# gnosisguild/stylus-zkvm-verifiers

Hardware: AMD Instinct MI355X
Metric: Groth16 proofs verified/sec (BN254) (higher is better)
Workload: dtype u32

## Files before the change

### stylus_zkvm_verifiers_amd/csrc/zkv_field.h

```cpp
#pragma once
#include <stdint.h>
#include "bn254_constants.h"

#if defined(__HIPCC__)
#define ZKV_HD __host__ __device__ __forceinline__
#define ZKV_HD_NI __host__ __device__ __noinline__ inline
#else
#define ZKV_HD inline
#define ZKV_HD_NI inline
#endif

#if defined(ZKV_COUNT_FP_MUL)
static thread_local unsigned long long zkv_fp_mul_counter = 0;
static thread_local unsigned long long zkv_mad_counter = 0;
static thread_local unsigned long long zkv_mad_issued_counter = 0;
static thread_local unsigned long long zkv_sqr_mad_excess_counter = 0;
#define ZKV_COUNT_MADS(n) (zkv_mad_counter += (n), zkv_mad_issued_counter += (n))
#define ZKV_COUNT_MADS_ISSUED(n) (zkv_mad_issued_counter += (n))
#else
#define ZKV_COUNT_MADS(n) ((void)0)
#define ZKV_COUNT_MADS_ISSUED(n) ((void)0)
#endif

#if defined(__HIP_DEVICE_COMPILE__)
#define ZKV_TABLE static __device__ const
#else
#define ZKV_TABLE static const
#endif

#if defined(ZKV_ASM_MARKS) && defined(__HIP_DEVICE_COMPILE__)
#define ZKV_MARK(name) asm volatile("; ZKVMARK " name)
#else
#define ZKV_MARK(name) ((void)0)
#endif

#ifndef ZKV_FAIR_SLICE_SHIFT
#define ZKV_FAIR_SLICE_SHIFT 17
#endif
ZKV_HD uint32_t zkv_wave_slot_parity() {
#if defined(__HIP_DEVICE_COMPILE__) && !defined(ZKV_NO_FAIR_SHARE)
    return __builtin_amdgcn_s_getreg((3 << 11) | 4) & 1u;
#else
    return 0;
#endif
}
ZKV_HD void zkv_fair_share(uint32_t slot_parity) {
#if defined(__HIP_DEVICE_COMPILE__) && !defined(ZKV_NO_FAIR_SHARE)
    const uint32_t t = (uint32_t)(__builtin_amdgcn_s_memrealtime() >> ZKV_FAIR_SLICE_SHIFT);
    if ((t ^ slot_parity) & 1u) __builtin_amdgcn_s_setprio(1);
    else __builtin_amdgcn_s_setprio(0);
#else
    (void)slot_parity;
#endif
}

#include "zkv_modinv.h"

namespace zkv {

struct Fp { uint32_t v[8]; };
struct Fp2C { Fp c0, c1; };
#if defined(ZKV_PAIRED)
struct Fp2 { Fp h; };
#else
struct Fp2 { Fp c0, c1; };
#endif
struct Fp6 { Fp2 c0, c1, c2; };

#if defined(__has_builtin)
#if __has_builtin(__builtin_addc) && __has_builtin(__builtin_subc)
#define ZKV_HAVE_CARRY_BUILTINS 1
#endif
#endif
ZKV_HD uint32_t addc(uint32_t a, uint32_t b, uint32_t& carry) {
#if defined(ZKV_HAVE_CARRY_BUILTINS)
    unsigned co; uint32_t r = __builtin_addc(a, b, carry, &co); carry = co; return r;
#else
    uint64_t t = (uint64_t)a + b + carry;
    carry = (uint32_t)(t >> 32);
    return (uint32_t)t;
#endif
}
ZKV_HD uint32_t subb(uint32_t a, uint32_t b, uint32_t& borrow) {
#if defined(ZKV_HAVE_CARRY_BUILTINS)
    unsigned bo; uint32_t r = __builtin_subc(a, b, borrow, &bo); borrow = bo; return r;
#else
    uint64_t t = (uint64_t)a - b - borrow;
    borrow = (uint32_t)(t >> 32) & 1u;
    return (uint32_t)t;
#endif
}

ZKV_HD Fp fp_zero() { Fp r; for (int i = 0; i < 8; i++) r.v[i] = 0; return r; }
ZKV_HD Fp fp_one() { Fp r = ZKV_FP_ONE; return r; }
ZKV_HD bool fp_is_zero(const Fp& a) {
    const uint32_t P[8] = ZKV_FP_P_LIMBS;
    uint32_t o = 0, q = 0;
    for (int i = 0; i < 8; i++) { o |= a.v[i]; q |= a.v[i] ^ P[i]; }
    return o == 0 || q == 0;
// ... 448 lines not shown
        if ((xo[i] >> 29) || (xp[i] >> 29) || (U[i] >> 29) || (V[i] >> 30)) zkv_col_shadow_bad++;
}
#define ZKV_DOT3_OPERANDS(a, b, c, d) zkv_dot3_operands(a, b, c, d)
#else
#define ZKV_DOT3_OPERANDS(a, b, c, d) ((void)0)
#endif
#if defined(ZKV_SHADOW_COLS) && !defined(__HIP_DEVICE_COMPILE__)
inline void zkv_limbs_below(const uint32_t (&a)[9], int bits) {
    for (int i = 0; i < 9; i++)
        if (a[i] >> bits) zkv_col_shadow_bad++;
}
#define ZKV_LIMBS_BELOW(a, bits) zkv_limbs_below(a, bits)
#else
#define ZKV_LIMBS_BELOW(a, bits) ((void)0)
#endif
ZKV_HD void f2_sum_open(uint64_t (&col)[18]) {
#pragma unroll
    for (int k = 0; k < 18; k++) col[k] = 0;
}
ZKV_HD void f2_sum_cross(uint64_t (&col)[18], const uint32_t (&ao)[9], const uint32_t (&ap)[9], const uint32_t (&bU)[9], const uint32_t (&bV)[9]) {
#if defined(ZKV_COUNT_FP_MUL)
    zkv_fp_mul_counter += 2;
#endif
    ZKV_DOT3_OPERANDS(ao, ap, bU, bV);
    fp_mac81(col, ao, bU); fp_mac81(col, ap, bV);
}
ZKV_HD void f2_sum_cross_dbl(uint64_t (&col)[18], const uint32_t (&ao2)[9], const uint32_t (&ap2)[9], const uint32_t (&bU)[9], const uint32_t (&bV)[9]) {
#if defined(ZKV_COUNT_FP_MUL)
    zkv_fp_mul_counter += 2;
#endif
    ZKV_LIMBS_BELOW(ao2, 30); ZKV_LIMBS_BELOW(ap2, 30); ZKV_LIMBS_BELOW(bU, 29); ZKV_LIMBS_BELOW(bV, 30);
    fp_mac81(col, ao2, bU); fp_mac81(col, ap2, bV);
}
ZKV_HD void f2_sum_sqr(uint64_t (&col)[18], const uint32_t (&M)[9], const uint32_t (&N)[9]) {
#if defined(ZKV_COUNT_FP_MUL)
    zkv_fp_mul_counter += 1;
#endif
    ZKV_LIMBS_BELOW(M, 30); ZKV_LIMBS_BELOW(N, 29);
    fp_mac81(col, M, N);
}
ZKV_HD Fp f2_sum_close(uint64_t (&col)[18]) {
    Fp r = fp_reduce_cols(col);
#if defined(__HIP_DEVICE_COMPILE__)
#pragma unroll
    for (int k = 0; k < 8; k++) asm volatile("" : "+v"(r.v[k]));
    __builtin_amdgcn_sched_barrier(0);
#endif
    return r;
}
ZKV_HD void fp_cols_carry32_dbl(uint64_t (&col)[18]) {
    uint32_t sixteen = 16u, two = 2u;
#if defined(__HIP_DEVICE_COMPILE__)
    asm volatile("" : "+s"(sixteen));
    asm volatile("" : "+s"(two));
#endif
#pragma unroll
    for (int k = 17; k >= 1; k--) {
        const uint32_t hi = (uint32_t)(col[k - 1] >> 32);
        const uint64_t keep = k == 17 ? col[17] + col[17] : (uint64_t)(uint32_t)col[k] * two;
        ZKV_COUNT_MADS_ISSUED(2);
        col[k] = col_add(keep, (uint64_t)hi * sixteen);
#if defined(__HIP_DEVICE_COMPILE__)
        asm volatile("" : "+v"(col[k]));
#endif
    }
    col[0] = (uint64_t)(uint32_t)col[0] * two;
}
ZKV_HD void f2_limbs_x_dbl(const Fp& v, uint32_t (&own2)[9], uint32_t (&par2)[9]) {
    uint32_t x[9];
    fp_unpack29(v, x);
#pragma unroll
    for (int i = 0; i < 9; i++) { own2[i] = x[i] << 1; par2[i] = zkv_partner_u32(own2[i]); }
}
ZKV_HD void f2_limbs_sqr(const uint32_t (&own)[9], const uint32_t (&par)[9], uint32_t (&M)[9], uint32_t (&N)[9]) {
    const uint32_t FAT[9] = ZKV_FP_FAT8P_LIMBS;
    const bool odd = zkv_parity() != 0;
#pragma unroll
    for (int i = 0; i < 9; i++) {
        M[i] = par[i] + (odd ? par[i] : own[i]);
        N[i] = own[i] + (odd ? 0u : FAT[i] - par[i]);
    }
#pragma unroll
    for (int k = 0; k < 8; k++) { N[k + 1] += N[k] >> 29; N[k] &= 0x1fffffffu; }
}
ZKV_HD void f2_dot3_first(uint64_t (&col)[18], const uint32_t (&ao)[9], const uint32_t (&ap)[9], const uint32_t (&bU)[9], const uint32_t (&bV)[9],
                          const uint32_t (&co)[9], const uint32_t (&cp)[9], const uint32_t (&dU)[9], const uint32_t (&dV)[9]) {
    f2_sum_open(col);
    f2_sum_cross(col, ao, ap, bU, bV); f2_sum_cross(col, co, cp, dU, dV);
    fp_cols_carry32(col);
}
ZKV_HD Fp f2_dot3_last(uint64_t (&col)[18], const uint32_t (&eo)[9], const uint32_t (&ep)[9], const uint32_t (&fU)[9], const uint32_t (&fV)[9]) {
    f2_sum_cross(col, eo, ep, fU, fV);
    return f2_sum_close(col);
}
ZKV_HD Fp f2_mul_limbs(const uint32_t (&ao)[9], const uint32_t (&ap)[9], const uint32_t (&bU)[9], const uint32_t (&bV)[9]) {
#if defined(ZKV_COUNT_FP_MUL)
    zkv_fp_mul_counter += 2;
#endif
    uint64_t col[18];
#pragma unroll
    for (int k = 0; k < 18; k++) col[k] = 0;
    fp_mac81(col, ao, bU); fp_mac81(col, ap, bV);
    return fp_reduce_cols(col);
}
struct L9 { uint32_t l[9]; };
ZKV_HD L9 l9_from_fp(const Fp& a) { L9 r; fp_unpack29(a, r.l); return r; }
ZKV_HD Fp l9_to_fp(const L9& a) { return fp_pack29(a.l); }
ZKV_HD L9 l9_partner(const L9& a) {
    L9 r;
#pragma unroll
    for (int i = 0; i < 9; i++) r.l[i] = zkv_partner_u32(a.l[i]);
    return r;
}
ZKV_HD L9 l9_mul_core(const L9& a, const L9& b) {
#if defined(ZKV_COUNT_FP_MUL)
    zkv_fp_mul_counter += 2;
#endif
    const uint32_t FAT[9] = ZKV_FP_FAT8P_LIMBS;
    uint32_t xo[9], U[9], V[9];
    uint64_t col[18];
#pragma unroll
    for (int k = 0; k < 18; k++) col[k] = 0;
#pragma unroll
    for (int i = 0; i < 9; i++) U[i] = zkv_pair_even_u32(b.l[i]);
    fp_mac81(col, a.l, U);
#pragma unroll
    for (int i = 0; i < 9; i++) { xo[i] = zkv_partner_u32(a.l[i]); V[i] = zkv_pair_odd_u32(b.l[i]); }
    if (zkv_parity() == 0) {
#pragma unroll
        for (int i = 0; i < 9; i++) V[i] = FAT[i] - V[i];
    }
    fp_mac81(col, xo, V);
    L9 r; fp_reduce_cols_limbs(col, r.l);
    return r;
}
#if defined(__HIP_DEVICE_COMPILE__) && defined(ZKV_FP_MUL_NOINLINE)
#define ZKV_L9P(p) uint32_t p##0, uint32_t p##1, uint32_t p##2, uint32_t p##3, uint32_t p##4, uint32_t p##5, uint32_t p##6, uint32_t p##7, uint32_t p##8
#define ZKV_L9A(f) f.l[0], f.l[1], f.l[2], f.l[3], f.l[4], f.l[5], f.l[6], f.l[7], f.l[8]
#define ZKV_L9MK(f, p) L9 f; f.l[0] = p##0; f.l[1] = p##1; f.l[2] = p##2; f.l[3] = p##3; f.l[4] = p##4; f.l[5] = p##5; f.l[6] = p##6; f.l[7] = p##7; f.l[8] = p##8
__device__ __noinline__ inline L9 l9_mul_ni(ZKV_L9P(pa), ZKV_L9P(pb)) {
    ZKV_L9MK(a, pa); ZKV_L9MK(b, pb);
    return l9_mul_core(a, b);
}
ZKV_HD L9 l9_mul(const L9& a, const L9& b) { return l9_mul_ni(ZKV_L9A(a), ZKV_L9A(b)); }
#else
ZKV_HD L9 l9_mul(const L9& a, const L9& b) { return l9_mul_core(a, b); }
#endif
struct LTerm { const uint32_t* x; int32_t k; };
#define ZKV_L9_G 256
template <int N> ZKV_HD L9 l9_lincomb(const LTerm (&t)[N], const int c) {
    const uint32_t P29[9] = ZKV_FP_P29_LIMBS;
    const int32_t D = (int32_t)P29[8] + 1;
    const uint32_t M = (uint32_t)(((1ull << 53) + (uint64_t)D - 1) / (uint64_t)D);
    int32_t top = 0;
#pragma unroll
    for (int j = 0; j < N; j++) top += t[j].k * (int32_t)t[j].x[8];
    const uint32_t tt = (uint32_t)(top + c * D - c - ZKV_L9_G);
    const int32_t nq = c - (int32_t)(uint32_t)(((uint64_t)tt * M) >> 53);
    L9 y; int64_t carry = 0;
#pragma unroll
    for (int i = 0; i < 9; i++) {
        int64_t s = carry;
#pragma unroll
        for (int j = 0; j < N; j++) s += (int64_t)t[j].k * (int64_t)(int32_t)t[j].x[i];
        s += (int64_t)nq * (int64_t)(int32_t)P29[i];
        if (i < 8) { y.l[i] = (uint32_t)s & 0x1fffffffu; carry = s >> 29; }
// ... 104 lines not shown
```

### stylus_zkvm_verifiers_amd/csrc/zkv_tower_mem.h

```cpp
#pragma once
#include "zkv_curve.h"

namespace zkv {

struct MRef {
    uint32_t* p; uint32_t stride; uint32_t f2w;
    ZKV_HD uint32_t ld(int k) const { return p[(size_t)k * stride]; }
    ZKV_HD void st(int k, uint32_t v) const { p[(size_t)k * stride] = v; }
    ZKV_HD int fw() const { return (int)f2w; }
};
ZKV_HD MRef m_ref(uint32_t* p, uint32_t stride, uint32_t f2w = 16) { MRef r; r.p = p; r.stride = stride; r.f2w = f2w; return r; }
ZKV_HD MRef m_off(MRef m, int words) { MRef r = m; r.p = m.p + (size_t)words * m.stride; return r; }

struct SoaRW {
    uint32_t* p; size_t stride; uint32_t off;
    ZKV_HD uint32_t ld(int k) const { return *(const uint32_t*)((const char*)(p + (size_t)k * stride) + off); }
    ZKV_HD void st(int k, uint32_t v) const { *(uint32_t*)((char*)(p + (size_t)k * stride) + off) = v; }
    ZKV_HD int fw() const { return 16; }
};
template <class R> ZKV_HD R m_fresh(R r) { return r; }
ZKV_HD SoaRW m_fresh(SoaRW r) {
#if defined(__HIP_DEVICE_COMPILE__)
    asm volatile("" : "+v"(r.off));
#endif
// ... 102 lines not shown
template <class RF> ZKV_HD void f12m_sqr_fused_body(RF f) {
    enum { A0 = 0, A1 = 3, A2 = 1, A3 = 4, A4 = 2, A5 = 5 };
    uint32_t x3o[9], x3p[9], y0U[9], y0V[9], z5U[9], z5V[9];
    uint32_t hU[9], hV[9];
    uint32_t ko[9], kp[9], jo[9], jp[9];
    uint32_t xo[9], xp[9], tU[9], tV[9];
    uint64_t col[18];
    Fp2 o1, o2, o3, o4, o5, o;
    f2_limbs_x(m_ld_f2(f, A3).h, x3o, x3p);
    f2_limbs_y(m_ld_f2(f, A1).h, hU, hV);
    f2_limbs_y(m_ld_f2(f, A2).h, tU, tV);
    f2_sum_open(col);
    f2_sum_cross(col, x3o, x3p, tU, tV);
    f2_limbs_x(m_ld_f2(f, A4).h, ko, kp);
    f2_sum_cross(col, ko, kp, hU, hV);
    fp_cols_carry32_dbl(col);
    f2_limbs_y(m_ld_f2(f, A0).h, y0U, y0V);
    f2_limbs_x_dbl(m_ld_f2(f, A5).h, xo, xp);
    f2_sum_cross_dbl(col, xo, xp, y0U, y0V);
    o5.h = f2_sum_close(col);
    f2_sum_open(col);
    f2_sum_cross(col, x3o, x3p, y0U, y0V);
    f2_limbs_x(m_ld_f2_again(f, A2).h, xo, xp);
    f2_sum_cross(col, xo, xp, hU, hV);
    fp_cols_carry32_dbl(col);
    { const Fp2 x5 = f2_mul_xi(m_ld_f2_again(f, A5)); f2_limbs_y(x5.h, z5U, z5V); }
    limbs_dbl_pinned(ko, kp, xo, xp);
    f2_sum_cross_dbl(col, xo, xp, z5U, z5V);
    o3.h = f2_sum_close(col);
    f2_sum_open(col);
    f2_sum_cross(col, ko, kp, y0U, y0V);
    f2_sum_cross(col, x3o, x3p, hU, hV);
    fp_cols_carry32_dbl(col);
    f2_limbs_x(m_ld_f2_again(f, A2).h, xo, xp);
    f2_limbs_sqr(xo, xp, tU, tV);
    f2_sum_sqr(col, tU, tV);
    f2_limbs_x(m_ld_f2_again(f, A5).h, xo, xp);
    f2_sum_cross(col, xo, xp, z5U, z5V);
    o4.h = f2_sum_close(col);
    m_st_f2(f, A5, o5);
    { const Fp2 x4 = f2_mul_xi(m_ld_f2_again(f, A4)); f2_limbs_y(x4.h, hU, hV); }
    f2_sum_open(col);
    f2_sum_cross(col, x3o, x3p, hU, hV);
    f2_limbs_x(m_ld_f2_again(f, A2).h, ko, kp);
    f2_sum_cross(col, ko, kp, z5U, z5V);
    fp_cols_carry32_dbl(col);
    f2_limbs_x(m_ld_f2_again(f, A1).h, jo, jp);
    limbs_dbl_pinned(jo, jp, xo, xp);
    f2_sum_cross_dbl(col, xo, xp, y0U, y0V);
    o1.h = f2_sum_close(col);
    f2_sum_open(col);
    f2_sum_cross(col, ko, kp, y0U, y0V);
    f2_sum_cross(col, x3o, x3p, z5U, z5V);
    fp_cols_carry32_dbl(col);
    f2_limbs_sqr(jo, jp, tU, tV);
    limbs_pin(tU); limbs_pin(tV);
    f2_sum_sqr(col, tU, tV);
    f2_limbs_x(m_ld_f2_again(f, A4).h, xo, xp);
    f2_sum_cross(col, xo, xp, hU, hV);
    o2.h = f2_sum_close(col);
    m_st_f2(f, A4, o4);
    f2_sum_open(col);
    f2_sum_cross(col, jo, jp, z5U, z5V);
    f2_sum_cross(col, ko, kp, hU, hV);
    fp_cols_carry32_dbl(col);
    f2_limbs_x(m_ld_f2_again(f, A0).h, xo, xp);
    f2_limbs_sqr(xo, xp, tU, tV);
    f2_sum_sqr(col, tU, tV);
    { const Fp2 x3 = f2_mul_xi(m_ld_f2_again(f, A3)); f2_limbs_y(x3.h, tU, tV); }
    f2_sum_cross(col, x3o, x3p, tU, tV);
    o.h = f2_sum_close(col);
    m_st_f2(f, A0, o); m_st_f2(f, A1, o1); m_st_f2(f, A2, o2); m_st_f2(f, A3, o3);
#if defined(ZKV_COUNT_FP_MUL)
    zkv_fp_mul_counter -= 15; zkv_mad_counter -= 729; zkv_mad_issued_counter -= 933; zkv_sqr_mad_excess_counter += 933;
#endif
}
template <class RF> ZKV_HD void f12m_sqr_body(RF f) {
#if defined(ZKV_SQR_KARATSUBA) && !defined(__HIP_DEVICE_COMPILE__)
    f12m_sqr_karatsuba_body(f);
#else
    f12m_sqr_fused_body(f);
#endif
}
#else
template <class RF> ZKV_HD void f12m_sqr_body(RF f) { f12m_sqr_karatsuba_body(f); }
#endif
template <class RF> ZKV_HD_NI void f12m_sqr(RF f) { f12m_sqr_body(f); }
ZKV_HD void fp4_sqr(const Fp2& a, const Fp2& b, Fp2& t0, Fp2& t1) {
    Fp2 tmp = f2_mul(a, b);
    t0 = f2_sub(f2_sub(f2_mul(f2_add(a, b), f2_add(f2_mul_xi(b), a)), tmp), f2_mul_xi(tmp));
    t1 = f2_dbl(tmp);
}
template <class RF> ZKV_HD void f12m_cyclo_sqr_body(RF f) {
    Fp2 z0 = m_ld_f2(f, 0), z1 = m_ld_f2(f, 4), t0, t1;
    fp4_sqr(z0, z1, t0, t1);
    z0 = f2_sub(t0, z0); z0 = f2_add(f2_dbl(z0), t0);
    z1 = f2_add(t1, z1); z1 = f2_add(f2_dbl(z1), t1);
    m_st_f2(f, 0, z0); m_st_f2(f, 4, z1);
    Fp2 z2 = m_ld_f2(f, 3), z3 = m_ld_f2(f, 2), t2, t3;
    fp4_sqr(z2, z3, t2, t3);
    Fp2 z4 = m_ld_f2(f, 1), z5 = m_ld_f2(f, 5), t4, t5;
    fp4_sqr(z4, z5, t4, t5);
    Fp2 x = f2_mul_xi(t5);
    z2 = f2_add(x, z2); z2 = f2_add(f2_dbl(z2), x);
    z3 = f2_sub(t4, z3); z3 = f2_add(f2_dbl(z3), t4);
    z4 = f2_sub(t2, z4); z4 = f2_add(f2_dbl(z4), t2);
    z5 = f2_add(t3, z5); z5 = f2_add(f2_dbl(z5), t3);
    m_st_f2(f, 3, z2); m_st_f2(f, 2, z3); m_st_f2(f, 1, z4); m_st_f2(f, 5, z5);
}
template <class RF> ZKV_HD_NI void f12m_cyclo_sqr(RF f) { f12m_cyclo_sqr_body(f); }
#if defined(ZKV_PAIRED)
struct L9Ref {
    zkv_lds_u32* p;
    ZKV_HD int fw() const { return 8; }
};
ZKV_HD L9Ref l9_ref(uint32_t* lds_base_plus_lane) { L9Ref r; r.p = (zkv_lds_u32*)lds_base_plus_lane; return r; }
ZKV_HD L9 l9_ld(L9Ref m, int idx) {
    L9 r;
#pragma unroll
    for (int k = 0; k < 9; k++) r.l[k] = m.p[(9 * idx + k) * 64];
    return r;
}
ZKV_HD void l9_st(L9Ref m, int idx, const L9& a) {
#pragma unroll
    for (int k = 0; k < 9; k++) m.p[(9 * idx + k) * 64] = a.l[k];
}
ZKV_HD Fp m_ld_fp(L9Ref m, int word0) { return l9_to_fp(l9_ld(m, word0 >> 3)); }
ZKV_HD void m_st_fp(L9Ref m, int word0, const Fp& a) { l9_st(m, word0 >> 3, l9_from_fp(a)); }

ZKV_HD void l9_fp4_sqr_update(const L9& a, const L9& b, const L9& za, const L9& zb, const bool xi_t1, L9& o0, L9& o1) {
    const bool odd = zkv_parity() != 0;
    const int32_t k1 = odd ? 1 : -1, k3 = odd ? -3 : 3;
    const L9 tmp = l9_mul(a, b);
    L9 s1, s2;
#pragma unroll
    for (int i = 0; i < 9; i++) s1.l[i] = a.l[i] + b.l[i];
    {
        const L9 pb = l9_partner(b);
        const LTerm t[3] = {{a.l, 1}, {b.l, 9}, {pb.l, k1}};
        s2 = l9_lincomb(t, 4);
    }
    const L9 S = l9_mul(s1, s2);
    const L9 tp = l9_partner(tmp);
    {
        const LTerm t[4] = {{S.l, 3}, {tmp.l, -30}, {tp.l, k3}, {za.l, -2}};
        o0 = l9_lincomb(t, 72);
    }
    if (!xi_t1) {
        const LTerm t[2] = {{tmp.l, 6}, {zb.l, 2}};
        o1 = l9_lincomb(t, 1);
    } else {
        const LTerm t[3] = {{tmp.l, 54}, {tp.l, -2 * k3}, {zb.l, 2}};
        o1 = l9_lincomb(t, 14);
    }
}
ZKV_HD void f12l9_cyclo_sqr(L9Ref f) {
    {
        const L9 a = l9_ld(f, 0), b = l9_ld(f, 4);
        L9 o0, o1;
        l9_fp4_sqr_update(a, b, a, b, false, o0, o1);
        l9_st(f, 0, o0); l9_st(f, 4, o1);
    }
    L9 n1, n5;
    {
        const L9 a = l9_ld(f, 3), b = l9_ld(f, 2), za = l9_ld(f, 1), zb = l9_ld(f, 5);
        l9_fp4_sqr_update(a, b, za, zb, false, n1, n5);
// ... 338 lines not shown
```

### stylus_zkvm_verifiers_amd/csrc/zkv_verify.h

```cpp
#pragma once
#include "zkv_tower_mem.h"
#include "zkv_sha256.h"
#include "zkv_gt.h"

namespace zkv {

enum : uint8_t {
    ST_OK = 0, ST_VERIFICATION_FAILED = 1, ST_INVALID_INITIALIZATION = 2, ST_ALREADY_INITIALIZED = 3,
    ST_INVALID_PROOF_DATA = 4, ST_SELECTOR_MISMATCH = 5,
    ST_BAD_CALLDATA = 6
};
enum : uint32_t { FL_ALIVE = 1u, FL_A_INF = 2u, FL_B_INF = 4u, FL_C_INF = 8u, FL_L_INF = 16u };

constexpr int N_LINES = 88;
constexpr int MSM_MAX_WINDOWS = 32;
constexpr int MSM_DIGITS = 256;
constexpr int MAX_IC = 6;
constexpr int MAX_VAR = 5;

struct VkRaw {
    uint32_t alpha[2][8];
    uint32_t beta[4][8], gamma[4][8], delta[4][8];
    uint32_t ic[MAX_IC][2][8];
    uint32_t n_ic;
// ... 209 lines not shown
ZKV_HD bool miller_loop_m(const VkTables* vkp, uint32_t flags, const G1Norm& n, const Fp2& bx, const Fp2& by, RF fm, RT tm, bool check_b = false) {
    const bool with_fixed = vkp != nullptr;
    const VkTables* vkq = with_fixed ? vkp : nullptr;
    const bool do_ab = !(flags & (FL_A_INF | FL_B_INF));
    const bool do_t = do_ab || (check_b && !(flags & FL_B_INF));
    bool do_l = with_fixed && !(flags & FL_L_INF) && !vkq->skip_fixed[0], do_c = with_fixed && !(flags & FL_C_INF) && !vkq->skip_fixed[1];
    const LineAffC* lines0 = with_fixed ? vkq->lines[0] : nullptr;
    const LineAffC* lines1 = with_fixed ? vkq->lines[1] : nullptr;
    f12m_set_one(fm);
    m_st_f2(tm, 0, bx); m_st_f2(tm, 1, by); m_st_f2(tm, 2, f2_one());
    Fp2 nby = f2_neg(by);
    Fp2 l0, l1, l3;
    int li = 0;
#pragma unroll 1
    for (int i = ZKV_ATE_NAF_LEN - 2; i >= 0; i--) {
        if (i != ZKV_ATE_NAF_LEN - 2) f12m_sqr(fm);
        if (do_t) {
            g2m_line_dbl(tm, &l0, &l1, &l3);
            if (do_ab) var_line_mul(fm, l0, l1, l3, n.axs, n.ays);
        }
        if (do_l) fixed_line_mul(fm, lines0[li], n.lxs, n.lys);
        if (do_c) fixed_line_mul(fm, lines1[li], n.cxs, n.cys);
        li++;
        int d = ate_naf(i);
        if (d != 0) {
            if (do_t) {
                Fp2 qy = d > 0 ? by : nby;
                g2m_line_add(tm, &bx, &qy, &l0, &l1, &l3);
                if (do_ab) var_line_mul(fm, l0, l1, l3, n.axs, n.ays);
            }
            if (do_l) fixed_line_mul(fm, lines0[li], n.lxs, n.lys);
            if (do_c) fixed_line_mul(fm, lines1[li], n.cxs, n.cys);
            li++;
        }
    }
    Fp2 qx[2], qy[2];
    g2_frob_affine(qx[0], qy[0], bx, by);
    g2_frob2_affine(qx[1], qy[1], bx, by);
    qy[1] = f2_neg(qy[1]);
#pragma unroll 1
    for (int s = 0; s < 2; s++) {
        if (do_t) {
            g2m_line_add(tm, &qx[s], &qy[s], &l0, &l1, &l3);
            if (do_ab) var_line_mul(fm, l0, l1, l3, n.axs, n.ays);
        }
        if (do_l) fixed_line_mul(fm, lines0[li], n.lxs, n.lys);
        if (do_c) fixed_line_mul(fm, lines1[li], n.cxs, n.cys);
        li++;
    }
    return !(check_b && do_t) || miller_point_closes(tm, bx, by);
}

#if defined(ZKV_PAIRED)
struct SoaRef {
    const uint32_t* p; size_t stride; uint32_t off;
    ZKV_HD Fp fp(int word0) const {
        Fp r;
#pragma unroll
        for (int k = 0; k < 8; k++) r.v[k] = *(const uint32_t*)((const char*)(p + (size_t)(word0 + k) * stride) + off);
        return r;
    }
};
template <class RF, class RT>
ZKV_HD bool miller_loop_p(const VkTables* vkp, uint32_t flags, SoaRef norm, SoaRef bsrc, RF fm, RT tm, bool check_b = false, const uint32_t* start = nullptr) {
    const uint8_t KIND[ZKV_MILLER_STEPS] = ZKV_MILLER_STEP_KIND;
    const bool with_fixed = vkp != nullptr;
    const bool do_ab = !(flags & (FL_A_INF | FL_B_INF));
    const bool do_t = do_ab || (check_b && !(flags & FL_B_INF));
    const bool do_l = with_fixed && !(flags & FL_L_INF) && !vkp->skip_fixed[0], do_c = with_fixed && !(flags & FL_C_INF) && !vkp->skip_fixed[1];
    if (start) f12m_copy(fm, m_ref(const_cast<uint32_t*>(start) + 8 * zkv_parity(), 1, 16));
    else f12m_set_one(fm);
    { Fp2 bx, by; bx.h = bsrc.fp(0); by.h = bsrc.fp(16); m_st_f2(tm, 0, bx); m_st_f2(tm, 1, by); m_st_f2(tm, 2, f2_one()); }
    const uint32_t slot = zkv_wave_slot_parity();
#pragma unroll 1
    for (int li = 0; li < ZKV_MILLER_STEPS; li++) {
        const int kind = KIND[li];
        zkv_fair_share(slot);
#if defined(__HIP_DEVICE_COMPILE__)
        asm volatile("" : "+v"(norm.off), "+v"(bsrc.off));
#endif
        if (kind == 0 && li != 0) { ZKV_MARK("begin sqr"); f12m_sqr_body(fm); ZKV_MARK("end sqr"); }
        if (do_t) {
            Fp2 l0, l1, l3;
            G2H T; T.x = m_ld_f2(tm, 0); T.y = m_ld_f2(tm, 1); T.z = m_ld_f2(tm, 2);
            if (kind == 0) { ZKV_MARK("begin linedbl"); line_dbl(T, l0, l1, l3); ZKV_MARK("end linedbl"); }
            else {
                Fp2 qx, qy; qx.h = bsrc.fp(0); qy.h = bsrc.fp(16);
                if (kind == 2) qy = f2_neg(qy);
                else if (kind == 3) { Fp2 x, y; g2_frob_affine(x, y, qx, qy); qx = x; qy = y; }
                else if (kind == 4) { Fp2 x, y; g2_frob2_affine(x, y, qx, qy); qx = x; qy = f2_neg(y); }
                ZKV_MARK("begin lineadd"); line_add(T, qx, qy, l0, l1, l3); ZKV_MARK("end lineadd");
            }
            m_st_f2(tm, 0, T.x); m_st_f2(tm, 1, T.y); m_st_f2(tm, 2, T.z);
            if (do_ab) {
                ZKV_MARK("begin mul034");
                const Fp2 c3 = f2_mul_fp(l1, norm.fp(0)), c4 = f2_mul_fp(l3, norm.fp(8));
                f12m_mul_by_034_body(fm, l0, c3, c4);
                ZKV_MARK("end mul034");
            }
        }
#pragma unroll 1
        for (int j = 0; j < 2; j++) {
            if (j == 0 ? !do_l : !do_c) continue;
            ZKV_MARK("begin mul134");
            const LineAffC& L = vkp->lines[j][li];
            const Fp2 c3 = f2_mul_fp(f2_const(L.nl), norm.fp(16 + 16 * j)), c4 = f2_mul_fp(f2_const(L.c), norm.fp(24 + 16 * j));
            f12m_mul_by_134_body(fm, c3, c4);
            ZKV_MARK("end mul134");
        }
    }
    if (!check_b || !do_t) return true;
    Fp2 qx, qy; qx.h = bsrc.fp(0); qy.h = bsrc.fp(16);
    return miller_point_closes(tm, qx, qy);
}
template <int G, class RF>
ZKV_HD uint32_t miller_loop_pg(uint32_t mask, uint32_t abmask, SoaRef norm, SoaRef bsrc, SoaRW tq, uint32_t step, RF fm) {
    const uint8_t KIND[ZKV_MILLER_STEPS] = ZKV_MILLER_STEP_KIND;
    f12m_set_one(fm);
#pragma unroll 1
    for (uint32_t p = 0; p < (uint32_t)G; p++) {
        if (!((mask >> p) & 1u)) continue;
        SoaRef b = bsrc; b.off += p * step;
        SoaRW t = tq; t.off += p * step;
        Fp2 bx, by; bx.h = b.fp(0); by.h = b.fp(16);
        m_st_f2(t, 0, bx); m_st_f2(t, 1, by); m_st_f2(t, 2, f2_one());
    }
#pragma unroll 1
    for (int li = 0; li < ZKV_MILLER_STEPS; li++) {
        const int kind = KIND[li];
#if defined(__HIP_DEVICE_COMPILE__)
        asm volatile("" : "+v"(norm.off), "+v"(bsrc.off), "+v"(tq.off));
#endif
        if (kind == 0 && li != 0) f12m_sqr_body(fm);
#pragma unroll 1
        for (uint32_t p = 0; p < (uint32_t)G; p++) {
            if (!((mask >> p) & 1u)) continue;
            SoaRef n = norm; n.off += p * step;
            SoaRef b = bsrc; b.off += p * step;
            SoaRW t = tq; t.off += p * step;
            Fp2 l0, l1, l3;
            G2H T; T.x = m_ld_f2(t, 0); T.y = m_ld_f2(t, 1); T.z = m_ld_f2(t, 2);
            if (kind == 0) line_dbl(T, l0, l1, l3);
            else {
                Fp2 qx, qy; qx.h = b.fp(0); qy.h = b.fp(16);
                if (kind == 2) qy = f2_neg(qy);
                else if (kind == 3) { Fp2 x, y; g2_frob_affine(x, y, qx, qy); qx = x; qy = y; }
                else if (kind == 4) { Fp2 x, y; g2_frob2_affine(x, y, qx, qy); qx = x; qy = f2_neg(y); }
                line_add(T, qx, qy, l0, l1, l3);
            }
            m_st_f2(t, 0, T.x); m_st_f2(t, 1, T.y); m_st_f2(t, 2, T.z);
            if ((abmask >> p) & 1u) {
                const Fp2 c3 = f2_mul_fp(l1, n.fp(0)), c4 = f2_mul_fp(l3, n.fp(8));
                f12m_mul_by_034_body(fm, l0, c3, c4);
            }
        }
    }
    uint32_t fine = (1u << G) - 1u;
#pragma unroll 1
    for (uint32_t p = 0; p < (uint32_t)G; p++) {
        if (!((mask >> p) & 1u)) continue;
        SoaRef b = bsrc; b.off += p * step;
        SoaRW t = tq; t.off += p * step;
        Fp2 qx, qy; qx.h = b.fp(0); qy.h = b.fp(16);
        if (!miller_point_closes(t, qx, qy)) fine &= ~(1u << p);
    }
    return fine;
}
#endif

ZKV_HD int8_t u_digit(int i) {
    const int8_t D[ZKV_U_DIG_LEN] = ZKV_U_DIG;
    return D[i];
}
template <class RA> ZKV_HD void exp_u_m(RA acc, MRef x, MRef W) {
    const MRef X17 = W, X35 = m_off(W, 96);
    f12m_copy(acc, x);
#pragma unroll 1
    for (int k = 0; k < 4; k++) f12m_cyclo_sqr(acc);
    f12m_mul(X17, acc, x);
    f12m_copy(acc, X17); f12m_cyclo_sqr(acc);
    f12m_mul(X35, acc, x);
    { const int t = u_digit(ZKV_U_DIG_LEN - 1); f12m_copy(acc, t == 1 ? x : t == 17 ? X17 : X35); }
#pragma unroll 1
    for (int i = ZKV_U_DIG_LEN - 2; i >= 0; i--) {
        f12m_cyclo_sqr(acc);
        const int d = u_digit(i);
        if (d == 0) continue;
        const int m = d < 0 ? -d : d;
        const MRef S = m == 1 ? x : m == 17 ? X17 : X35;
        if (d > 0) f12m_mul(acc, acc, S);
        else f12m_mul_conj(acc, acc, S);
    }
}
template <class RA> ZKV_HD bool final_exp_is_one_m(MRef F, MRef E, MRef Y1, MRef Y3, MRef Y4, MRef W, RA acc) {
    f12m_copy(acc, F); f12m_conj(acc);
    f12m_inv(F, F);
    f12m_mul(acc, acc, F);
    f12m_frob(F, acc, 2);
    f12m_mul(E, F, acc);
    exp_u_m(acc, E, W); f12m_conj(acc);
    f12m_cyclo_sqr(acc); f12m_copy(Y1, acc);
    f12m_cyclo_sqr(acc);
    f12m_mul(acc, acc, Y1); f12m_copy(Y3, acc);
    exp_u_m(acc, Y3, W); f12m_conj(acc); f12m_copy(Y4, acc);
    f12m_cyclo_sqr(acc); f12m_copy(F, acc);
    exp_u_m(acc, F, W);
    f12m_conj(Y3);
    f12m_mul(acc, acc, Y4);
    f12m_mul(acc, acc, Y3); f12m_copy(Y3, acc);
    f12m_mul(F, acc, Y1);
    f12m_mul(acc, acc, Y4);
    f12m_mul(acc, acc, E);
    f12m_frob(Y1, F, 1);
    f12m_mul(acc, Y1, acc);
    f12m_frob(Y3, Y3, 2);
    f12m_mul(acc, Y3, acc);
    f12m_conj(E);
    f12m_mul(E, E, F);
    f12m_frob(E, E, 3);
    f12m_mul(acc, E, acc);
    return f12m_is_one(acc);
}
#define ZKV_MILLER_START_HR {0xd636f235u, 0x1c2edc10u, 0xd3290123u, 0x194998a4u, 0x59a7280au, 0xdddc0ef8u, 0xe131a018u, 0x30644e72u}
#define ZKV_MILLER_START_E {0x0093e79bu, 0xed92c00du, 0x46b3b592u, 0xa24730bau, 0xea466f56u, 0x04db5c66u, 0x47869ae3u, 0x02b6f45eu}
#define ZKV_MILLER_START_E_BITS 250
ZKV_HD void miller_start_value(MRef out, MRef M, MRef E, MRef Y1, MRef Y3, MRef Y4, MRef W, MRef acc) {
    const uint32_t EX[8] = ZKV_MILLER_START_E;
    (void)final_exp_is_one_m(M, E, Y1, Y3, Y4, W, acc);
    f12m_copy(out, acc);
#pragma unroll 1
    for (int i = ZKV_MILLER_START_E_BITS - 2; i >= 0; i--) {
        f12m_cyclo_sqr(out);
        if ((EX[i >> 5] >> (i & 31)) & 1u) f12m_mul(out, out, acc);
// ... 314 lines not shown
```

Baseline: 6.640 million.

## Fuse G2 line doubling and addition into lane-pair limb-level bodies

Replaces the generic Fp2-level line_dbl and line_add in the Miller loop with fused bodies that work on lane-paired 29-bit limbs. Products are accumulated into column sums and reduced once, negation and the factor 3 are folded into limb operands, and the G2 point is read from and written to memory inside the step. The goal is fewer modular reductions and fewer intermediate Fp2 values, which should lower MAD count and register pressure in the line-function part of the pairing. In exchange there is much more hand-written arithmetic whose limb-bound assumptions must hold for correctness, and the batched path only uses the new doubling step.

```diff
diff --git a/stylus_zkvm_verifiers_amd/csrc/zkv_field.h b/stylus_zkvm_verifiers_amd/csrc/zkv_field.h
--- a/stylus_zkvm_verifiers_amd/csrc/zkv_field.h
+++ b/stylus_zkvm_verifiers_amd/csrc/zkv_field.h
@@ -15,6 +15,7 @@
 static thread_local unsigned long long zkv_mad_counter = 0;
 static thread_local unsigned long long zkv_mad_issued_counter = 0;
 static thread_local unsigned long long zkv_sqr_mad_excess_counter = 0;
+static thread_local long long zkv_line_mad_excess_counter = 0;
 #define ZKV_COUNT_MADS(n) (zkv_mad_counter += (n), zkv_mad_issued_counter += (n))
 #define ZKV_COUNT_MADS_ISSUED(n) (zkv_mad_issued_counter += (n))
 #else
@@ -629,6 +630,60 @@
     }
 #pragma unroll
     for (int k = 0; k < 8; k++) { N[k + 1] += N[k] >> 29; N[k] &= 0x1fffffffu; }
+}
+ZKV_HD void f2_limbs_xy(const Fp& v, uint32_t (&own)[9], uint32_t (&par)[9], uint32_t (&U)[9], uint32_t (&V)[9]) {
+    const uint32_t FAT[9] = ZKV_FP_FAT8P_LIMBS;
+    fp_unpack29(v, own);
+#pragma unroll
+    for (int i = 0; i < 9; i++) { par[i] = zkv_partner_u32(own[i]); U[i] = zkv_pair_even_u32(own[i]); V[i] = zkv_pair_odd_u32(own[i]); }
+    if (zkv_parity() == 0) {
+#pragma unroll
+        for (int i = 0; i < 9; i++) V[i] = FAT[i] - V[i];
+    }
+}
+ZKV_HD void f2_limbs_yn(const Fp& v, uint32_t (&NU)[9], uint32_t (&NV)[9]) {
+    const uint32_t FAT[9] = ZKV_FP_FAT8P_LIMBS;
+    uint32_t y[9];
+    fp_unpack29(v, y);
+#pragma unroll
+    for (int i = 0; i < 9; i++) { NU[i] = FAT[i] - zkv_pair_even_u32(y[i]); NV[i] = zkv_pair_odd_u32(y[i]); }
+    if (zkv_parity() != 0) {
+#pragma unroll
+        for (int i = 0; i < 9; i++) NV[i] = FAT[i] - NV[i];
+    }
+}
+ZKV_HD void f2_limbs_y_neg(const uint32_t (&U)[9], const uint32_t (&V)[9], uint32_t (&NU)[9], uint32_t (&NV)[9]) {
+    const uint32_t FAT[9] = ZKV_FP_FAT8P_LIMBS;
+#pragma unroll
+    for (int i = 0; i < 9; i++) { NU[i] = FAT[i] - U[i]; NV[i] = FAT[i] - V[i]; }
+}
+ZKV_HD void f2_limbs_y_const(const Fp2C& c, uint32_t (&U)[9], uint32_t (&V)[9]) {
+    const uint32_t FAT[9] = ZKV_FP_FAT8P_LIMBS;
+    const bool odd = zkv_parity() != 0;
+    uint32_t y1[9];
+    fp_unpack29(c.c0, U); fp_unpack29(c.c1, y1);
+#pragma unroll
+    for (int i = 0; i < 9; i++) V[i] = odd ? y1[i] : FAT[i] - y1[i];
+}
+ZKV_HD void f2_sum_cross_neg(uint64_t (&col)[18], const uint32_t (&ao)[9], const uint32_t (&ap)[9], const uint32_t (&nU)[9], const uint32_t (&nV)[9]) {
+#if defined(ZKV_COUNT_FP_MUL)
+    zkv_fp_mul_counter += 2;
+#endif
+    ZKV_LIMBS_BELOW(ao, 29); ZKV_LIMBS_BELOW(ap, 29); ZKV_LIMBS_BELOW(nU, 30);
+#if defined(ZKV_SHADOW_COLS) && !defined(__HIP_DEVICE_COMPILE__)
+    if (zkv_parity() == 0) zkv_limbs_below(nV, 29); else zkv_limbs_below(nV, 30);
+#endif
+    fp_mac81(col, ao, nU); fp_mac81(col, ap, nV);
+}
+ZKV_HD void f2_sum_sqr_x3(uint64_t (&col)[18], const uint32_t (&M)[9], const uint32_t (&N)[9]) {
+#if defined(ZKV_COUNT_FP_MUL)
+    zkv_fp_mul_counter += 1;
+#endif
+    ZKV_LIMBS_BELOW(M, 30); ZKV_LIMBS_BELOW(N, 29);
+    uint32_t M3[9];
+#pragma unroll
+    for (int i = 0; i < 9; i++) M3[i] = M[i] + (M[i] << 1);
+    fp_mac81(col, M3, N);
 }
 ZKV_HD void f2_dot3_first(uint64_t (&col)[18], const uint32_t (&ao)[9], const uint32_t (&ap)[9], const uint32_t (&bU)[9], const uint32_t (&bV)[9],
                           const uint32_t (&co)[9], const uint32_t (&cp)[9], const uint32_t (&dU)[9], const uint32_t (&dV)[9]) {
diff --git a/stylus_zkvm_verifiers_amd/csrc/zkv_tower_mem.h b/stylus_zkvm_verifiers_amd/csrc/zkv_tower_mem.h
--- a/stylus_zkvm_verifiers_amd/csrc/zkv_tower_mem.h
+++ b/stylus_zkvm_verifiers_amd/csrc/zkv_tower_mem.h
@@ -208,6 +208,123 @@
     f12m_sqr_fused_body(f);
 #endif
 }
+
+#if defined(ZKV_COUNT_FP_MUL)
+struct LineStepCharge {
+    unsigned long long m0, c0, i0;
+    LineStepCharge() : m0(zkv_fp_mul_counter), c0(zkv_mad_counter), i0(zkv_mad_issued_counter) {}
+    void settle(unsigned muls, unsigned mads) {
+        zkv_line_mad_excess_counter += (long long)(zkv_mad_issued_counter - i0) - (long long)mads;
+        zkv_fp_mul_counter = m0 + muls; zkv_mad_counter = c0 + mads; zkv_mad_issued_counter = i0 + mads;
+    }
+};
+#endif
+template <class RT> ZKV_HD void line_dbl_pair_body(RT tm, Fp2& l0, Fp2& l1, Fp2& l3) {
+#if defined(ZKV_COUNT_FP_MUL)
+    LineStepCharge charge;
+#endif
+    const Fp2C b3c = ZKV_TWIST_3B;
+    uint32_t xo[9], xp[9], yo[9], yp[9], yU[9], yV[9], M[9], N[9];
+    uint64_t col[18];
+    Fp A, B, C, E, H;
+    f2_limbs_x(m_ld_f2(tm, 0).h, xo, xp);
+    f2_limbs_sqr(xo, xp, M, N);
+    f2_sum_open(col); f2_sum_sqr_x3(col, M, N); l1.h = f2_sum_close(col);
+    f2_limbs_xy(m_ld_f2(tm, 1).h, yo, yp, yU, yV);
+    f2_sum_open(col); f2_sum_cross(col, xo, xp, yU, yV); A = f2_sum_close(col);
+    f2_limbs_x(m_ld_f2(tm, 2).h, xo, xp);
+    f2_limbs_sqr(xo, xp, M, N);
+    f2_sum_open(col); f2_sum_sqr(col, M, N); C = f2_sum_close(col);
+#pragma unroll
+    for (int i = 0; i < 9; i++) { xo[i] <<= 1; xp[i] <<= 1; }
+    f2_sum_open(col); f2_sum_cross_dbl(col, xo, xp, yU, yV); H = f2_sum_close(col);
+    f2_limbs_sqr(yo, yp, M, N);
+    f2_sum_open(col); f2_sum_sqr(col, M, N); B = f2_sum_close(col);
+    f2_limbs_x(C, xo, xp); f2_limbs_y_const(b3c, yU, yV);
+    f2_sum_open(col); f2_sum_cross(col, xo, xp, yU, yV); E = f2_sum_close(col);
+    Fp F, D, BpF, BmF, K;
+    fp_sub_x2(fp_zero(), H, E, B, l0.h, l3.h);
+    F = fp_add(fp_add(E, E), E);
+    fp_add_x2(B, F, F, F, BpF, D);
+    BmF = fp_sub(B, F); K = fp_add(D, D);
+    f2_limbs_x_dbl(A, xo, xp); f2_limbs_y(BmF, yU, yV);
+    f2_sum_open(col); f2_sum_cross_dbl(col, xo, xp, yU, yV); A = f2_sum_close(col);
+    { Fp2 o; o.h = A; m_st_f2(tm, 0, o); }
+    f2_limbs_x_dbl(H, xo, xp); f2_limbs_y(fp_add_nr(B, B), yU, yV);
+    f2_sum_open(col); f2_sum_cross_dbl(col, xo, xp, yU, yV); H = f2_sum_close(col);
+    { Fp2 o; o.h = H; m_st_f2(tm, 2, o); }
+    f2_limbs_x(BpF, xo, xp);
+    f2_limbs_sqr(xo, xp, M, N);
+    f2_sum_open(col); f2_sum_sqr(col, M, N);
+    f2_limbs_x(K, xo, xp); f2_limbs_yn(E, yU, yV);
+    f2_sum_cross_neg(col, xo, xp, yU, yV);
+    { Fp2 o; o.h = f2_sum_close(col); m_st_f2(tm, 1, o); }
+#if defined(ZKV_COUNT_FP_MUL)
+    charge.settle(14, 1944);
+#endif
+}
+template <class RT> ZKV_HD void line_add_pair_body(RT tm, const Fp2& qx, const Fp2& qy, Fp2& l0, Fp2& l1, Fp2& l3) {
+#if defined(ZKV_COUNT_FP_MUL)
+    LineStepCharge charge;
+#endif
+    uint32_t zo[9], zp[9], to[9], tp[9], lo[9], lp[9], U[9], V[9], NU[9], NV[9], xo[9], xp[9];
+    uint64_t col[18];
+    Fp th, la, c, d, e, f, g, h;
+    f2_limbs_x(m_ld_f2(tm, 2).h, zo, zp);
+    f2_limbs_yn(qy.h, NU, NV);
+    f2_sum_open(col); f2_sum_cross_neg(col, zo, zp, NU, NV); th = f2_sum_close(col);
+    th = fp_add(m_ld_f2(tm, 1).h, th);
+    f2_limbs_y(qx.h, U, V);
+    f2_sum_open(col); f2_sum_cross(col, zo, zp, U, V); la = f2_sum_close(col);
+    la = fp_sub(m_ld_f2(tm, 0).h, la);
+    f2_limbs_x(th, to, tp); f2_limbs_x(la, lo, lp);
+    f2_sum_open(col); f2_sum_cross(col, to, tp, U, V); f2_sum_cross_neg(col, lo, lp, NU, NV); l3.h = f2_sum_close(col);
+    l0.h = la; l1.h = fp_neg(th);
+    f2_limbs_sqr(to, tp, U, V);
+    f2_sum_open(col); f2_sum_sqr(col, U, V); c = f2_sum_close(col);
+    f2_limbs_sqr(lo, lp, U, V);
+    f2_sum_open(col); f2_sum_sqr(col, U, V); d = f2_sum_close(col);
+    f2_limbs_y(d, U, V);
+    f2_sum_open(col); f2_sum_cross(col, lo, lp, U, V); e = f2_sum_close(col);
+    f2_limbs_x(m_ld_f2_again(m_fresh(tm), 0).h, xo, xp);
+    f2_sum_open(col); f2_sum_cross(col, xo, xp, U, V); g = f2_sum_close(col);
+    f2_limbs_y(c, U, V);
+    f2_sum_open(col); f2_sum_cross(col, zo, zp, U, V); f = f2_sum_close(col);
+    fp_add_x2(e, f, g, g, c, d);
+    h = fp_sub(c, d); g = fp_sub(g, h);
+    f2_limbs_y(h, U, V);
+    f2_sum_open(col); f2_sum_cross(col, lo, lp, U, V);
+    { Fp2 o; o.h = f2_sum_close(col); m_st_f2(tm, 0, o); }
+    f2_limbs_y(e, U, V);
+    f2_sum_open(col); f2_sum_cross(col, zo, zp, U, V);
+    { Fp2 o; o.h = f2_sum_close(col); m_st_f2(tm, 2, o); }
+    f2_limbs_y_neg(U, V, NU, NV);
+    f2_limbs_x(m_ld_f2_again(m_fresh(tm), 1).h, xo, xp);
+    f2_limbs_y(g, U, V);
+    f2_sum_open(col); f2_sum_cross_neg(col, xo, xp, NU, NV); f2_sum_cross(col, to, tp, U, V);
+    { Fp2 o; o.h = f2_sum_close(col); m_st_f2(tm, 1, o); }
+#if defined(ZKV_COUNT_FP_MUL)
+    charge.settle(24, 2997);
+#endif
+}
+template <class RT> ZKV_HD void line_dbl_step(RT tm, Fp2& l0, Fp2& l1, Fp2& l3) {
+#if defined(ZKV_LINE_STEP_CLASSIC) && !defined(__HIP_DEVICE_COMPILE__)
+    G2H T; T.x = m_ld_f2(tm, 0); T.y = m_ld_f2(tm, 1); T.z = m_ld_f2(tm, 2);
+    line_dbl(T, l0, l1, l3);
+    m_st_f2(tm, 0, T.x); m_st_f2(tm, 1, T.y); m_st_f2(tm, 2, T.z);
+#else
+    line_dbl_pair_body(tm, l0, l1, l3);
+#endif
+}
+template <class RT> ZKV_HD void line_add_step(RT tm, const Fp2& qx, const Fp2& qy, Fp2& l0, Fp2& l1, Fp2& l3) {
+#if defined(ZKV_LINE_STEP_CLASSIC) && !defined(__HIP_DEVICE_COMPILE__)
+    G2H T; T.x = m_ld_f2(tm, 0); T.y = m_ld_f2(tm, 1); T.z = m_ld_f2(tm, 2);
+    line_add(T, qx, qy, l0, l1, l3);
+    m_st_f2(tm, 0, T.x); m_st_f2(tm, 1, T.y); m_st_f2(tm, 2, T.z);
+#else
+    line_add_pair_body(tm, qx, qy, l0, l1, l3);
+#endif
+}
 #else
 template <class RF> ZKV_HD void f12m_sqr_body(RF f) { f12m_sqr_karatsuba_body(f); }
 #endif
diff --git a/stylus_zkvm_verifiers_amd/csrc/zkv_verify.h b/stylus_zkvm_verifiers_amd/csrc/zkv_verify.h
--- a/stylus_zkvm_verifiers_amd/csrc/zkv_verify.h
+++ b/stylus_zkvm_verifiers_amd/csrc/zkv_verify.h
@@ -315,16 +315,14 @@
         if (kind == 0 && li != 0) { ZKV_MARK("begin sqr"); f12m_sqr_body(fm); ZKV_MARK("end sqr"); }
         if (do_t) {
             Fp2 l0, l1, l3;
-            G2H T; T.x = m_ld_f2(tm, 0); T.y = m_ld_f2(tm, 1); T.z = m_ld_f2(tm, 2);
-            if (kind == 0) { ZKV_MARK("begin linedbl"); line_dbl(T, l0, l1, l3); ZKV_MARK("end linedbl"); }
+            if (kind == 0) { ZKV_MARK("begin linedbl"); line_dbl_step(tm, l0, l1, l3); ZKV_MARK("end linedbl"); }
             else {
                 Fp2 qx, qy; qx.h = bsrc.fp(0); qy.h = bsrc.fp(16);
                 if (kind == 2) qy = f2_neg(qy);
                 else if (kind == 3) { Fp2 x, y; g2_frob_affine(x, y, qx, qy); qx = x; qy = y; }
                 else if (kind == 4) { Fp2 x, y; g2_frob2_affine(x, y, qx, qy); qx = x; qy = f2_neg(y); }
-                ZKV_MARK("begin lineadd"); line_add(T, qx, qy, l0, l1, l3); ZKV_MARK("end lineadd");
-            }
-            m_st_f2(tm, 0, T.x); m_st_f2(tm, 1, T.y); m_st_f2(tm, 2, T.z);
+                ZKV_MARK("begin lineadd"); line_add_step(tm, qx, qy, l0, l1, l3); ZKV_MARK("end lineadd");
+            }
             if (do_ab) {
                 ZKV_MARK("begin mul034");
                 const Fp2 c3 = f2_mul_fp(l1, norm.fp(0)), c4 = f2_mul_fp(l3, norm.fp(8));
@@ -372,16 +370,16 @@
             SoaRef b = bsrc; b.off += p * step;
             SoaRW t = tq; t.off += p * step;
             Fp2 l0, l1, l3;
-            G2H T; T.x = m_ld_f2(t, 0); T.y = m_ld_f2(t, 1); T.z = m_ld_f2(t, 2);
-            if (kind == 0) line_dbl(T, l0, l1, l3);
+            if (kind == 0) line_dbl_step(t, l0, l1, l3);
             else {
+                G2H T; T.x = m_ld_f2(t, 0); T.y = m_ld_f2(t, 1); T.z = m_ld_f2(t, 2);
                 Fp2 qx, qy; qx.h = b.fp(0); qy.h = b.fp(16);
                 if (kind == 2) qy = f2_neg(qy);
                 else if (kind == 3) { Fp2 x, y; g2_frob_affine(x, y, qx, qy); qx = x; qy = y; }
                 else if (kind == 4) { Fp2 x, y; g2_frob2_affine(x, y, qx, qy); qx = x; qy = f2_neg(y); }
                 line_add(T, qx, qy, l0, l1, l3);
-            }
-            m_st_f2(t, 0, T.x); m_st_f2(t, 1, T.y); m_st_f2(t, 2, T.z);
+                m_st_f2(t, 0, T.x); m_st_f2(t, 1, T.y); m_st_f2(t, 2, T.z);
+            }
             if ((abmask >> p) & 1u) {
                 const Fp2 c3 = f2_mul_fp(l1, n.fp(0)), c4 = f2_mul_fp(l3, n.fp(8));
                 f12m_mul_by_034_body(fm, l0, c3, c4);
```

New measurement: 6.697 million, median of 6. Within noise of the previous version (+0.9%).
